# Yujia-Yan/Transkun

Hardware: AMD Instinct MI355X
Metric: semi-CRF logProb+backward steps/sec at T=1024, NBatch=352 (higher is better)
Workload: dtype f32; 1 GPU; NeuralSemiCRFInterval(score, noise).logProb(intervals) fwd+bwd through the public API (Python interval lists packed inside the timed region), T=1024, NBatch=352 per GPU, fp32, exact-hash randn-like scores resident in HBM; T=1024, NBatch=352, impl=0, parallelism=chains sharded, 1 rank(s) seen by the process group, no data-path collective

## Files before the change

transkun_amd/csrc/persist.hip:

```cpp
#include <atomic>
#include <stdlib.h>
#include "common.h"
#include "pathscore.h"

#ifndef SEMICRF_PANEL_PROBES
#define SEMICRF_PANEL_PROBES 0
#endif

#ifndef SEMICRF_PROBE_TASKS
#define SEMICRF_PROBE_TASKS 0
#endif
#ifndef SEMICRF_PROBE_HIST
#define SEMICRF_PROBE_HIST 0
#endif

#ifndef SEMICRF_CT_DBG
#define SEMICRF_CT_DBG -1
#endif

namespace semicrf {

constexpr int PB = 16;
#ifndef SEMICRF_RING
#define SEMICRF_RING 4
// ... 59 lines not shown
constexpr int CTRL_COPYQ = 192;
constexpr int CTRL_PATHQ = 160;
constexpr int CTRL_GEN = 96;

typedef unsigned long long u64;
typedef unsigned v4u __attribute__((ext_vector_type(4)));
typedef unsigned v4u_a4 __attribute__((ext_vector_type(4), aligned(4)));
template <int V>
struct IC { static constexpr int value = V; };

#define DBGF(P) (SEMICRF_CT_DBG >= 0 ? (unsigned)SEMICRF_CT_DBG : (P).dbg)
struct SweepParams {
    const float* score;
    const float* noise;
    int T, B, K;
    int c0, c1;
    int nSpine, nPanelGroups;
    int nTasks;
    int taskBase;
    int panelWaves;
    int hybridPanelWaves;
    int hybridStart;
    int zeroWaves;
    unsigned tag;
    int selfclean;
    unsigned expect_gen;
    unsigned dbg;
    unsigned* ctrl;
    u64* ts;
    unsigned* ug;
    unsigned* ug_other;
    int gradLazyShort;
    int bandWaves;
    u64* farg;
    float* u_out;
    float* last_out;
    int* code;
    const float* vfwd;
    const float* logZ;
    const float* gout;
    int gstride;
    float gscale;
    float* dScore;
    float* dNoise;
    const int* pathPairs;
    const int* pathOffsets;
    int pathK;
    int pathSpine;
    float* pathOut;
    u64* pathg;
    float noiseAdd;
    float* band;
    unsigned* bandFlags;
    int bandSpines;
    int bandGroups;
    int bandK0;
    int copyWaves;
    int cellNT;
    int gradNT;
    int nfarw;
};

__device__ __forceinline__ float fexp2(float x) { return __builtin_amdgcn_exp2f(x); }
__device__ __forceinline__ float flog2(float x) { return __builtin_amdgcn_logf(x); }

__device__ __forceinline__ u64 make_granule(unsigned tag, float v)
// ... 68 lines not shown
}

__device__ __forceinline__ bool spin_abort(unsigned* ctrl, int& spins, int limit, unsigned code)
{
    ++spins;
    if (spins > limit) { set_error(ctrl, code); s_abort = 1; return true; }
    if ((spins & 255) == 0 &&
        __hip_atomic_load(ctrl + 1, __ATOMIC_RELAXED, __HIP_MEMORY_SCOPE_AGENT) != CTRL_INIT) { s_abort = 1; return true; }
    return false;
}

#ifndef SEMICRF_NLOADER
#define SEMICRF_NLOADER 1
#endif
constexpr int NLOADER = SEMICRF_NLOADER;
#ifndef SEMICRF_NRBUF
#define SEMICRF_NRBUF 4
#endif
constexpr int NRBUF = SEMICRF_NRBUF;
constexpr int TILE_BYTES = PB * PB * RS * 4;
constexpr int NCONST = 3;
constexpr int LDS_TILES = 0;
constexpr int LDS_CONST = LDS_TILES + NRBUF * RING * TILE_BYTES;
constexpr int LDS_FAR = LDS_CONST + NRBUF * NCONST * 256;
constexpr int NFAR = 8;
constexpr int NPOS = 128;
static_assert(NFAR >= RING && NPOS >= RING * PB, "ring geometry");
constexpr int LDS_RING = LDS_FAR + NFAR * 64 * 16;
#ifndef SEMICRF_STAGGER
#define SEMICRF_STAGGER 32
#endif
#ifndef SEMICRF_GRAD_LAZY
#define SEMICRF_GRAD_LAZY 127
#endif
#ifndef SEMICRF_GRAD_HSTART
#define SEMICRF_GRAD_HSTART 12
#endif
#ifndef SEMICRF_LOADER_PACE
#define SEMICRF_LOADER_PACE 0
#endif
#ifndef SEMICRF_LOADER_AUX
#define SEMICRF_LOADER_AUX 0
#endif
#ifndef SEMICRF_SPH
#define SEMICRF_SPH 1
#endif
#ifndef SEMICRF_FAR_EARLY
#define SEMICRF_FAR_EARLY 0
#endif
#ifndef SEMICRF_FAR_PRIO
#define SEMICRF_FAR_PRIO 0
#endif
#ifndef SEMICRF_NFARW
#define SEMICRF_NFARW 2
#endif
constexpr int NFARW = SEMICRF_NFARW;
constexpr int NNSLOT = 8;
constexpr int NEAR_SLOT_BYTES = NNEAR * TILE_BYTES + 256;
constexpr int LDS_NEAR = LDS_RING + NPOS * RS * 8;
constexpr int LDS_CTL = LDS_NEAR + (NNEAR > 0 ? NNSLOT * NEAR_SLOT_BYTES : 0);
static_assert(NPOS >= (FAR0 + 1) * PB && NNSLOT >= FAR0 + 1 && NRBUF + RING + NNSLOT + NFARW <= 64 && NNSLOT % NFARW == 0, "near geometry");
constexpr int LDS_DUMMY = LDS_CTL + 256;
constexpr int LDS_SPINE_BYTES = LDS_DUMMY + (64 * 2 + PB * 8) * 4;

typedef __attribute__((address_space(3))) void lds_void_t;
typedef __attribute__((address_space(1))) const void gbl_void_t;
// ... 259 lines not shown
            if (lane == 0) lds_flag_store(fcons, k + 1);
        }
        if (fprobe && k < 64) P.ts[704 + k] = __builtin_amdgcn_s_memrealtime();
        if (NNEAR > 0) {
            const int own0 = k * PB;
            const unsigned bvoff = DIR == 0 ? (unsigned)(((size_t)(prow_c - own0) * T * Bs + cc) * 4)
                                            : (unsigned)(((size_t)(T - 1 - prow_c) * Bs + cc) * 4);
#pragma unroll
            for (int n = NNEAR - 1; n >= 0; --n) {
                const int b = k - RING - n;
                if (b < 0) continue;
                float uq[PB];
#pragma unroll
                for (int u4 = 0; u4 < PB; u4 += 4) {
                    const int j = b * PB + u4;
                    const float* e = rd_base + (j % NPOS) * 8;
                    u64 w0, w1, w2, w3;
                    int spins = 0;
                    while (true) {
                        w0 = lds_load64(e); w1 = lds_load64(e + 2 * RS); w2 = lds_load64(e + 4 * RS); w3 = lds_load64(e + 6 * RS);
                        if (__all((int)(w0 >> 32) == j + 1 && (int)(w1 >> 32) == j + 2 && (int)(w2 >> 32) == j + 3 && (int)(w3 >> 32) == j + 4)) break;
                        __builtin_amdgcn_s_sleep(1);
                        if (spin_abort(ctrl, spins, SPIN_LIMIT_LDS, 12)) break;
                    }
                    uq[u4] = __uint_as_float((unsigned)w0); uq[u4 + 1] = __uint_as_float((unsigned)w1);
                    uq[u4 + 2] = __uint_as_float((unsigned)w2); uq[u4 + 3] = __uint_as_float((unsigned)w3);
                }
                if (fprobe && k < 64 && n == 0) P.ts[768 + k] = __builtin_amdgcn_s_memrealtime();
                if (MODE == 0) {
                    float t[PB];
#pragma unroll
                    for (int u = 0; u < PB; ++u) {
                        t[u] = fmaf(ncell[n][u], LOG2E, uq[u]);
                        if (GRAD && rvalid && P.bandWaves == 0) {
                            const int j = b * PB + u;
                            const size_t co = DIR == 0 ? ((size_t)own0 * T + (size_t)j) * Bs : (size_t)(T - 1 - j) * T * Bs;
                            const auto rs = __builtin_amdgcn_make_buffer_rsrc((void*)(dScore + co), 0, 0x7fffffff, 0x00020000);
                            __builtin_amdgcn_raw_buffer_store_b32(__float_as_uint(gz * fexp2(t[u] + arow)), rs, bvoff, 0, 0);
                        }
                    }
                    float mx = aM;
#pragma unroll
                    for (int u = 0; u < PB; u += 2) mx = fmaxf(mx, fmaxf(t[u], t[u + 1]));
                    float sum = aS * fexp2(aM - mx);
#pragma unroll
                    for (int u = 0; u < PB; ++u) sum += fexp2(t[u] - mx);
                    aM = mx; aS = sum;
                } else {
#pragma unroll
                    for (int u = 0; u < PB; ++u) max_push_sel(aM, aK, uq[u] + ncell[n][u], frame_of<DIR>(b * PB + u, T));
                }
            }
        }
        if (fprobe && k < 64) P.ts[832 + k] = __builtin_amdgcn_s_memrealtime();
        if (rvalid && nparts > 0) {
            for (int p0 = 0; p0 < nparts; p0 += 4) {
                const int np = nparts - p0 < 4 ? nparts - p0 : 4;
                u64 gq[4];
                bool have[4] = {false, false, false, false};
                int spins = 0;
                bool first = SEMICRF_FAR_EARLY && p0 == 0;
                while (true) {
#pragma unroll
                    for (int i = 0; i < 4; ++i)
                        if (i < np && !have[i])
                            gq[i] = first ? eq[i] : load_granule(farg + ((size_t)(p0 + i) * T + prow) * Bs + c);
                    first = false;
// ... 322 lines not shown
            if (GRAD)
                dScore[((size_t)frow * T + frow) * Bs + c] = gz * fexp2(arow + mine + draw - 2.0f * sp);
            if (MODE == 1) code[(size_t)c * T + frow] = (mykey + 1) | (sp > 0.0f ? 0x40000000 : 0);
        }
        if (SEMICRF_PANEL_PROBES && trace) ts[k] = __builtin_amdgcn_s_memrealtime();
    }
}

#ifndef SEMICRF_GRAD_AUX
#define SEMICRF_GRAD_AUX 2
#endif
constexpr int GRAD_AUX = SEMICRF_GRAD_AUX;
#ifndef SEMICRF_CELL_AUX
#define SEMICRF_CELL_AUX 2
#endif
constexpr int CELL_AUX = SEMICRF_CELL_AUX;
#ifndef SEMICRF_PNS
#define SEMICRF_PNS 3
#endif
constexpr int PNS = SEMICRF_PNS;
constexpr int PSTAGE_BYTES = 10240;
#ifndef SEMICRF_PW_MAX
#define SEMICRF_PW_MAX 5
#endif
constexpr int PW_MAX = SEMICRF_PW_MAX;
constexpr int LDS_PANEL_BYTES = PW_MAX * PNS * PSTAGE_BYTES;
constexpr int SPH = SEMICRF_SPH;
constexpr int HWAVES = SPH == 1 ? RING + NLOADER + 1 : RING + NLOADER + NFARW;
constexpr int LDS_HALF = (LDS_SPINE_BYTES + 1023) / 1024 * 1024;
constexpr int LDS_HYBRID_PANEL = SPH * LDS_HALF;
constexpr int HPW_MAX = (160 * 1024 - 512 - LDS_HYBRID_PANEL) / (PNS * PSTAGE_BYTES) < NT / 64 - SPH * HWAVES
                            ? (160 * 1024 - 512 - LDS_HYBRID_PANEL) / (PNS * PSTAGE_BYTES) : NT / 64 - SPH * HWAVES;
static_assert(SPH * HWAVES <= NT / 64 && SPH * LDS_HALF <= 160 * 1024 - 512 && (GP / GS) % SPH == 0, "wave roles");
constexpr int LDS_HYBRID_BYTES = LDS_HYBRID_PANEL + (HPW_MAX > 0 ? HPW_MAX : 0) * PNS * PSTAGE_BYTES;
constexpr int LDS_DYN_MAX2 = SPH * LDS_HALF > LDS_PANEL_BYTES ? SPH * LDS_HALF : LDS_PANEL_BYTES;
constexpr int LDS_DYN_BYTES = LDS_HYBRID_BYTES > LDS_DYN_MAX2 ? LDS_HYBRID_BYTES : LDS_DYN_MAX2;
__device__ __forceinline__ void acc_lift(float& M, float& S, float tm)
{
    const bool need = tm > M + (RESC_HI - RESC_EARLY);
    const float newM = need ? floorf(tm) + RESC_LIFT : M;
    const int sh = (int)fmaxf(M - newM, -4096.0f);
    S = __builtin_ldexpf(S, sh);
    M = newM;
}

struct PanelGeom {
    int pirow[4];
    unsigned voff;
    unsigned fvoff;
    unsigned gvoff;
};

template <int DIR>
__device__ __forceinline__ size_t panel_tile_off(const PanelGeom& G, int m, int T, size_t Bs)
{
    return DIR == 0 ? ((size_t)G.pirow[0] * T + (size_t)m * PB) * Bs
                    : ((size_t)(T - 1 - (m * PB + 15)) * T + (size_t)(T - 1 - G.pirow[3])) * Bs;
}
template <int DIR>
__device__ __forceinline__ unsigned panel_soff(const PanelGeom& G, int rr, int h, int T, size_t Bs)
{
    return DIR == 0 ? (unsigned)((((size_t)(G.pirow[rr] - G.pirow[0]) * T + 8 * h) * Bs) * 4)
                    : (unsigned)((((size_t)(1 - h) * 8 * T + (G.pirow[3] - G.pirow[rr])) * Bs) * 4);
}
template <bool COHERENT>
__device__ __forceinline__ void panel_fetch_gran(__amdgpu_buffer_rsrc_t ursrc, char* stage, unsigned gvoff, int m, int B)
// ... 231 lines not shown
                            else __builtin_amdgcn_s_sleep(SEMICRF_GRAD_LAZY);
                        }
                        else __builtin_amdgcn_s_sleep(16);
                        if (spin_abort(ctrl, spins, SPIN_LIMIT, 5)) break;
                        ++npoll;
                        if (m == q) panel_fetch_gran<true>(ursrc, stage, G.gvoff, m, B);
                        const unsigned pw = __builtin_amdgcn_raw_buffer_load_b32(ursrc, (unsigned)(cl * 4), (unsigned)((m * PB + PB - 1) * B * 4), 16);
                        if (!__all(pw != U_EMPTY || !cvalid)) continue;
                        if (m != q) panel_fetch_gran<true>(ursrc, stage, G.gvoff, m, B);
                        wait_vmcnt<0>();
                        panel_read_gran(grbase + (unsigned)(s * PSTAGE_BYTES), g0, g1);
                    }
                }
                if (frontier && m + 1 < m1) {
                    const int sn = s + 1 == PNS ? 0 : s + 1;
                    panel_fetch_gran<true>(ursrc, stage0 + sn * PSTAGE_BYTES, G.gvoff, m + 1, B);
                    issued += 2;
                    if (sn == 0) mark0 = issued; else if (sn == 1) mark1 = issued; else mark2 = issued;
                }
                if (SEMICRF_PANEL_PROBES && (dbg & 16u) && g == 0 && q4 == 0 && m == q && lane == 0) P.ts[192 + k] = __builtin_amdgcn_s_memrealtime();
                if (c >= c1) { g0.x = 0u; g1.x = 0u; }
                if (c + 1 >= c1) { g0.y = 0u; g1.y = 0u; }
                if (c + 2 >= c1) { g0.z = 0u; g1.z = 0u; }
                if (c + 3 >= c1) { g0.w = 0u; g1.w = 0u; }
                const float uv[2][4] = {{__uint_as_float(g0.x), __uint_as_float(g0.y), __uint_as_float(g0.z), __uint_as_float(g0.w)},
                                        {__uint_as_float(g1.x), __uint_as_float(g1.y), __uint_as_float(g1.z), __uint_as_float(g1.w)}};

                if (MODE == 0) {
                    typedef float v2f __attribute__((ext_vector_type(2)));
                    const v2f l2e = {LOG2E, LOG2E};
                    const v2f u2[2][2] = {{{uv[0][0], uv[0][1]}, {uv[0][2], uv[0][3]}}, {{uv[1][0], uv[1][1]}, {uv[1][2], uv[1][3]}}};
                    const auto gs = __builtin_amdgcn_make_buffer_rsrc((void*)(GRAD ? dScore + panel_tile_off<DIR>(G, m, T, Bs) : nullptr), 0,
                                                                      0x7fffffff, 0x00020000);
#pragma unroll
                    for (int rr = 0; rr < 4; ++rr) {
                        v2f e[2][2];
#pragma unroll
                        for (int h = 0; h < 2; ++h) {
                            const v4u xv = xo[rr * 2 + h];
                            const v2f x2[2] = {{__uint_as_float(xv.x), __uint_as_float(xv.y)}, {__uint_as_float(xv.z), __uint_as_float(xv.w)}};
#pragma unroll
                            for (int j = 0; j < 2; ++j) {
                                const v2f mj = {aM[rr][2 * j], aM[rr][2 * j + 1]};
                                e[h][j] = __builtin_elementwise_fma(x2[j], l2e, u2[h][j] - mj);
                            }
                        }
                        const float emax = fmaxf(fmaxf(fmaxf(e[0][0].x, e[0][0].y), fmaxf(e[0][1].x, e[0][1].y)),
                                                 fmaxf(fmaxf(e[1][0].x, e[1][0].y), fmaxf(e[1][1].x, e[1][1].y)));
                        if (__any(emax > RESC_HI)) {
#pragma unroll
                            for (int i = 0; i < 4; ++i) {
                                const float x0 = __uint_as_float(i == 0 ? xo[rr * 2].x : (i == 1 ? xo[rr * 2].y : (i == 2 ? xo[rr * 2].z : xo[rr * 2].w)));
                                const float x1 = __uint_as_float(i == 0 ? xo[rr * 2 + 1].x : (i == 1 ? xo[rr * 2 + 1].y : (i == 2 ? xo[rr * 2 + 1].z : xo[rr * 2 + 1].w)));
                                const float t0 = fmaf(x0, LOG2E, uv[0][i]), t1 = fmaf(x1, LOG2E, uv[1][i]);
                                acc_lift(aM[rr][i], aS[rr][i], fmaxf(t0, t1));
                                const float e0 = t0 - aM[rr][i], e1 = t1 - aM[rr][i];
                                if (i & 1) { e[0][i >> 1].y = e0; e[1][i >> 1].y = e1; } else { e[0][i >> 1].x = e0; e[1][i >> 1].x = e1; }
                            }
                        }
                        v2f mg[2][2];
#pragma unroll
                        for (int j = 0; j < 2; ++j) {
                            v2f sj = {aS[rr][2 * j], aS[rr][2 * j + 1]};
                            const v2f p0 = {fexp2(e[0][j].x), fexp2(e[0][j].y)};
                            const v2f p1 = {fexp2(e[1][j].x), fexp2(e[1][j].y)};
                            sj = (sj + p0) + p1;
                            aS[rr][2 * j] = sj.x; aS[rr][2 * j + 1] = sj.y;
                            if (GRAD) {
                                const v2f mj = {aM[rr][2 * j], aM[rr][2 * j + 1]};
                                const v2f aj = {arow[rr][2 * j], arow[rr][2 * j + 1]};
                                const v2f fa = mj + aj;
                                const v2f gzj = {gz[2 * j], gz[2 * j + 1]};
                                const v2f fx = {fexp2(fa.x), fexp2(fa.y)};
                                const v2f gF = gzj * fx;
                                mg[0][j] = gF * p0;
                                mg[1][j] = gF * p1;
                            }
                        }
                        if (GRAD) {
#pragma unroll
                            for (int h = 0; h < 2; ++h) {
                                if (cvalid && pbase + rr < T) {
                                    const unsigned so = panel_soff<DIR>(G, rr, h, T, Bs);
                                    v4u gv;
                                    gv.x = __float_as_uint(mg[h][0].x);
                                    gv.y = __float_as_uint(mg[h][0].y);
                                    gv.z = __float_as_uint(mg[h][1].x);
                                    gv.w = __float_as_uint(mg[h][1].y);
#ifdef SEMICRF_NO_PANEL_GSTORE
                                    asm volatile("" ::"v"(gv));
                                    continue;
#endif
                                    if (c + 3 < c1) {
                                        if (grad_nt) __builtin_amdgcn_raw_buffer_store_b128(gv, gs, G.voff, so, GRAD_AUX);
                                        else __builtin_amdgcn_raw_buffer_store_b128(gv, gs, G.voff, so, 0);
                                    }
                                    else {
                                        __builtin_amdgcn_raw_buffer_store_b32(gv.x, gs, G.voff, so, 0);
                                        if (c + 1 < c1) __builtin_amdgcn_raw_buffer_store_b32(gv.y, gs, G.voff + 4, so, 0);
                                        if (c + 2 < c1) __builtin_amdgcn_raw_buffer_store_b32(gv.z, gs, G.voff + 8, so, 0);
                                    }
                                }
                            }
                        }
                        __builtin_amdgcn_sched_barrier(0);
                    }
                    if (GRAD) issued += nst;
                } else {
#pragma unroll
                    for (int rr = 0; rr < 4; ++rr)
#pragma unroll
                        for (int h = 0; h < 2; ++h) {
                            const v4u xv = xo[rr * 2 + h];
                            const float xe[4] = {__uint_as_float(xv.x), __uint_as_float(xv.y), __uint_as_float(xv.z), __uint_as_float(xv.w)};
                            const int key = frame_of<DIR>(m * PB + slot + 8 * h, T);
#pragma unroll
                            for (int i = 0; i < 4; ++i) max_push_seq<DIR>(aM[rr][i], aK[rr][i], uv[h][i] + xe[i], key);
                        }
                }
            }
            if (tprobe) { P.ts[1664 + k] = __builtin_amdgcn_s_memrealtime(); P.ts[1792 + k] = (u64)npoll; }
            if (refill) {
                panel_fetch_cells<DIR>(score, G, stage, m + PNS, T, Bs, cell_nt);
                if (!probe_stream && !probe_nou) panel_fetch_gran<false>(ursrc, stage, G.gvoff, m + PNS, B);
                issued += 10;
                if (s == 0) mark0 = issued; else if (s == 1) mark1 = issued; else mark2 = issued;
            }
        }
        if (tr) { tsp[2] = __builtin_amdgcn_s_memrealtime(); tsp[4] = (u64)(m1 - m0) | ((u64)k << 8) | ((u64)(frontier ? 1 : 0) << 16) | ((u64)part << 20); }
        if (!(GRAD && MODE == 0)) wait_vmcnt<0>();
        (void)frontier;
        if (SEMICRF_PANEL_PROBES && (dbg & 16u) && g == 0 && q4 == 0 && m1 == q + 1 && lane == 0 && k < 64 && T >= 1024)
            P.ts[1728 + k] = __builtin_amdgcn_s_memrealtime();

        const bool b5 = (lane & 32) != 0, b4 = (lane & 16) != 0, b3 = (lane & 8) != 0;
        u64* fbase = farg + (size_t)part * T * Bs;
        const int pi = pbase + (b5 ? 2 : 0) + (b4 ? 1 : 0);
        {
            constexpr int RSTR = 65 * 8;
            char* const rb = stage0;
// ... 54 lines not shown
    if (tail0 + lane < n) rowp[tail0 + lane] = 0.f;
}
__device__ __forceinline__ void zero_role(const SweepParams& P)
{
    const int T = P.T, B = P.B;
    float* const dScore = P.dScore;
    unsigned* const ctrl = P.ctrl;
    const int lane = threadIdx.x & 63;
    const int npairs = T / 2;
    while (true) {
        int p = 0;
        if (lane == 0) p = (int)(atomicAdd(ctrl + 3, 1u) + 1u);
        p = __builtin_amdgcn_readfirstlane(p);
        if (p >= npairs) break;
        const int e2 = T - 2 - p;
        if (p <= e2) zero_row(dScore, p, T, B, lane);
        if (p < e2) zero_row(dScore, e2, T, B, lane);
    }
}

constexpr int CTRL_BANDQ = 32;

template <int DIR>
__device__ __forceinline__ void band_role(const SweepParams& P)
{
    const int T = P.T, B = P.B, K = P.K, c0 = P.c0, c1 = P.c1;
    const size_t Bs = (size_t)B;
    unsigned* const ctrl = P.ctrl;
    const float* __restrict__ score = P.score;
    float* const dScore = P.dScore;
    const int lane = threadIdx.x & 63;
    const int q8 = lane & 7, pjsub = (lane >> 3) & 1, pisub = lane >> 4;
    const int nG = P.nPanelGroups;
    const int nTasks = K * FAR0 * nG * 4;
    const size_t last4 = (size_t)T * T * Bs - 4;
    const auto ursrc = __builtin_amdgcn_make_buffer_rsrc((void*)P.ug, 0, (int)((size_t)T * Bs * 4), 0x00020000);
    const bool grad_nt = __builtin_amdgcn_readfirstlane(P.gradNT) != 0;
    while (true) {
        int task = 0;
        if (lane == 0) task = (int)(atomicAdd(ctrl + CTRL_BANDQ, 1u) + 1u);
        task = __builtin_amdgcn_readfirstlane(task);
        if (task >= nTasks) break;
        const int q4 = task & 3, t2 = task >> 2;
        const int g = t2 % nG, t3 = t2 / nG;
        const int dk = t3 % FAR0, m = t3 / FAR0, k = m + dk;
        const int pbase = k * PB + q4 * 4;
        if (k >= K || pbase >= T) continue;
#if defined(SEMICRF_BAND_ABL) && SEMICRF_BAND_ABL == 2
        continue;
#endif
        const int pi = pbase + pisub;
        const bool rowok = pi < T;
        const int pic = rowok ? pi : T - 1;
        const int c = c0 + g * GP + q8 * 4;
        const int cl = c < c1 ? c : c0;
        const bool v0 = c < c1, v1 = c + 1 < c1, v2 = c + 2 < c1, v3 = c + 3 < c1;
        float gz[4], ar[4];
        {
            const int fr = frame_of<DIR>(pic, T);
#pragma unroll
            for (int i = 0; i < 4; ++i) {
                const bool ok = c + i < c1;
                const float lz = ok ? P.logZ[c + i] : 0.f;
                gz[i] = ok ? P.gout[(size_t)(c + i) * P.gstride] * P.gscale : 0.f;
                ar[i] = ok ? (P.vfwd[(size_t)fr * Bs + c + i] - lz) * LOG2E : 0.f;
            }
        }
        v4u x[8], uu[8];
        size_t off[8];
        unsigned uoff[8];
        bool use[8];
#pragma unroll
        for (int e = 0; e < 8; ++e) {
            const int pj = m * PB + 2 * e + pjsub;
            use[e] = rowok && pj < pi;
            const int pjc = pj < pic ? pj : (pic > 0 ? pic - 1 : 0);
            off[e] = cell_index<DIR>(pic, pjc, T) * Bs + cl;
            uoff[e] = (unsigned)(((size_t)pjc * Bs + cl) * 4);
// ... 91 lines not shown

template <int MODE, int DIR, bool GRAD>
__global__ __launch_bounds__(NT) void persist_sweep_kernel(SweepParams P)
{
    extern __shared__ __attribute__((aligned(16))) char s_dyn[];
    __shared__ int s_exit;
    if (threadIdx.x == 0) {
        const unsigned e1 = __hip_atomic_load(P.ctrl + 1, __ATOMIC_RELAXED, __HIP_MEMORY_SCOPE_AGENT);
        const unsigned gen = P.selfclean ? __hip_atomic_load(P.ctrl + CTRL_GEN, __ATOMIC_RELAXED, __HIP_MEMORY_SCOPE_AGENT) : P.expect_gen;
        s_abort = e1 != CTRL_INIT ? 1 : 0;
        if (gen != P.expect_gen) { set_error(P.ctrl, 13u); s_abort = 1; }
        s_exit = 0;
    }
    for (int h = 0; h < SPH; ++h)
        for (int i = threadIdx.x; i < (LDS_DUMMY - LDS_FAR) / 4; i += NT) ((int*)(s_dyn + h * LDS_HALF + LDS_FAR))[i] = 0;
    __syncthreads();
    const int nSpineWG = (P.nSpine + SPH - 1) / SPH;
    const int ticket = wg_ticket(nSpineWG, (int)gridDim.x, (int)blockIdx.x);
    const int wave = (int)(threadIdx.x >> 6);
    if (P.ug_other && wave == NT / 64 - 1) {
        const size_t n = (size_t)P.T * P.B, n4 = n / 4;
        const size_t per = (n4 + gridDim.x - 1) / gridDim.x, i0 = per * blockIdx.x, i1 = i0 + per < n4 ? i0 + per : n4;
        const v4u e = {U_EMPTY, U_EMPTY, U_EMPTY, U_EMPTY};
        for (size_t i = i0 + (threadIdx.x & 63); i < i1; i += 64) ((v4u*)P.ug_other)[i] = e;
        if (blockIdx.x == 0 && (threadIdx.x & 63) < (int)(n - n4 * 4)) P.ug_other[n4 * 4 + (threadIdx.x & 63)] = U_EMPTY;
    }
    const bool clk = SEMICRF_PANEL_PROBES && (DBGF(P) & 128u) && ticket == nSpineWG + 3 && threadIdx.x == 0;
    if (clk) { P.ts[600] = __builtin_readcyclecounter(); P.ts[601] = __builtin_amdgcn_s_memrealtime(); }
    if (SEMICRF_PROBE_HIST && (DBGF(P) & 1024u) && threadIdx.x == 0) {
        const unsigned long long now = (unsigned long long)__builtin_amdgcn_s_memrealtime();
        atomicMin((unsigned long long*)(P.ts + (3 * P.T) / 2), now);
        atomicMin((unsigned long long*)(P.ts + (3 * P.T) / 2 + 129 + (__builtin_amdgcn_s_getreg(6164) & 7)), now);
    }
    if (ticket < nSpineWG) {
        const int half = wave / HWAVES, hw = wave % HWAVES;
        const int sg = ticket * SPH + half;
        char* const lds_h = s_dyn + half * LDS_HALF;
        if (half >= SPH) {
            const int xw = wave - SPH * HWAVES;
            if (SPH == 1 && NFARW > 1 && wave >= NT / 64 - (NFARW - 1)) {
                if (ticket < P.nSpine && !(DBGF(P) & 9u)) far_role<MODE, DIR, GRAD>(P, ticket, s_dyn, 1 + wave - (NT / 64 - (NFARW - 1)));
            } else if (!(DBGF(P) & 2u) && xw < P.hybridPanelWaves) {
                {
                    const int* cons = (const int*)(s_dyn + LDS_CTL) + NRBUF;
                    int spins = 0;
                    while (lds_flag_load(cons + (P.hybridStart % RING)) < P.hybridStart + 1 && P.hybridStart < P.K &&
                           !(SEMICRF_PANEL_PROBES && (DBGF(P) & 8u))) {
                        __builtin_amdgcn_s_sleep(127);
                        if (spin_abort(P.ctrl, spins, SPIN_LIMIT_LDS, 10)) break;
                    }
                }
                panel_role<MODE, DIR, GRAD>(P, s_dyn + LDS_HYBRID_PANEL, xw, 1);
            } else if (MODE == 0 && DIR == 0 && !GRAD && P.pathPairs != nullptr && P.pathSpine && xw == P.hybridPanelWaves) {
                path_role(P);
            }
        } else if (sg >= P.nSpine) {
        } else if (hw < RING) {
            if (!(DBGF(P) & 8u)) {
                if (GRAD && P.bandWaves == 0) spine_role<MODE, DIR, GRAD, GRAD>(P, sg, hw, lds_h);
                else spine_role<MODE, DIR, GRAD, false>(P, sg, hw, lds_h);
            }
        } else if (hw < RING + NLOADER) {
            if (!(DBGF(P) & 8u)) loader_role<DIR, GRAD>(P, sg, lds_h, hw - RING);
        } else {
            if (!(DBGF(P) & 9u)) far_role<MODE, DIR, GRAD>(P, sg, lds_h, hw - (RING + NLOADER));
        }
    } else {
        if (!(DBGF(P) & 2u) && wave < P.panelWaves)
            panel_role<MODE, DIR, GRAD>(P, s_dyn, wave, 0, P.taskBase > 0 ? (ticket - nSpineWG) * P.panelWaves + wave : -1);
        else if (GRAD && wave - P.panelWaves >= 0 && wave - P.panelWaves < P.zeroWaves) zero_role(P);
        else if (GRAD && wave - P.panelWaves - P.zeroWaves >= 0 && wave - P.panelWaves - P.zeroWaves < P.bandWaves) band_role<DIR>(P);
        else if (SEMICRF_BANDX && wave >= NT / 64 - P.copyWaves && (ticket - nSpineWG) % SEMICRF_BANDX_WGSTRIDE == 0) copy_role<DIR>(P);
        else if (MODE == 0 && DIR == 0 && !GRAD && P.pathPairs != nullptr && wave == P.panelWaves) path_role(P);
    }
    if (clk) { P.ts[602] = __builtin_readcyclecounter(); P.ts[603] = __builtin_amdgcn_s_memrealtime(); }
    if (P.selfclean) {
        int left = 0;
        if ((threadIdx.x & 63) == 0) left = atomicAdd(&s_exit, 1) + 1;
        left = __builtin_amdgcn_readfirstlane(left);
        if (left == NT / 64) {
            unsigned before = 0;
            if ((threadIdx.x & 63) == 0) before = atomicAdd(P.ctrl + CTRL_EXIT, 1u) + 1u;
            before = (unsigned)__builtin_amdgcn_readfirstlane((int)before);
            if (before + 1u == gridDim.x &&
                __hip_atomic_load(P.ctrl + 1, __ATOMIC_RELAXED, __HIP_MEMORY_SCOPE_AGENT) == CTRL_INIT) {
                for (int i = threadIdx.x & 63; i < (int)CTRL_WORDS; i += 64)
                    __hip_atomic_store(P.ctrl + i, i == CTRL_GEN ? P.tag : CTRL_INIT, __ATOMIC_RELAXED, __HIP_MEMORY_SCOPE_AGENT);
            }
        }
    }
}

template <int DIR>
__device__ __forceinline__ void band_copy_load(const float* __restrict__ score, int T, int B, int kr, int g, int t, int q, int lane,
                                               v4u_a4 (&v)[8])
{
    const int q8 = lane & 7, cs = lane >> 3;
    const int cbase = (g * (GP / GS) + q8) * GS;
    const size_t Bs = (size_t)B;
    const size_t last4 = (size_t)T * T * Bs - 4;
    const int kc = kr - t > 0 ? kr - t : 0;
#pragma unroll
    for (int it = 0; it < 8; ++it) {
        const int ci = q * 64 + it * 8 + cs;
        const int col = ci >> 4, tr = ci & 15;
        const int prow_t = kr * PB + tr < T ? kr * PB + tr : T - 1;
        int pj = kc * PB + col;
// ... 134 lines not shown
    static std::atomic<int> ncu[MAX_DEVICES];
    const int dev = current_device();
    int n = ncu[dev].load();
    if (n == 0) {
        int v = 0;
        n = 256;
        if (hipDeviceGetAttribute(&v, hipDeviceAttributeMultiprocessorCount, dev) == hipSuccess && v > 0) n = v;
        ncu[dev].store(n);
    }
    return n;
}

size_t persist_workspace_bytes(int T, int B)
{
    return CTRL_BYTES + align_up((size_t)2 * T * sizeof(u64)) + (size_t)max_parts(T) * align_up((size_t)T * B * sizeof(u64)) +
           2 * align_up((size_t)T * B * sizeof(unsigned)) +
           align_up((size_t)B * sizeof(u64)) +
           band_flag_bytes(T, B) + band_copy_bytes(T, B);
}

bool persist_supported(int T, int B)
{
    return B >= 2 && T >= 2 && T < 65535 && (long long)T * B * 64 < (1ll << 31) &&
           (B + GS - 1) / GS <= MAX_CHUNKS * (device_cus() / 2 > 0 ? device_cus() / 2 : 1);
}

static unsigned next_tag()
{
    static std::atomic<unsigned> counter{0};
    const unsigned lo = (counter.fetch_add(1) % 65534u) + 1u;
    return (lo << 16) | lo;
}

struct Knobs { int hybrid_waves, hybrid_start, panel_waves, zero_waves, band_waves, nfarw; };
static Knobs read_knobs()
{
#if defined(SEMICRF_DEBUG_BUILD) && SEMICRF_DEBUG_BUILD
    auto get = [](const char* name) { const char* e = getenv(name); return e ? atoi(e) : -1; };
    return Knobs{get("SEMICRF_HYBRID_PANEL_WAVES"), get("SEMICRF_HYBRID_START"), get("SEMICRF_PANEL_WAVES"), get("SEMICRF_ZERO_WAVES"),
                 get("SEMICRF_BAND_WAVES"), get("SEMICRF_NFARW_RT")};
#else
    return Knobs{-1, -1, -1, -1, -1, -1};
#endif
}

struct GradArgs {
    const float* vfwd; const float* logZ; const float* gout; float* dScore; float* dNoise; int gstride; float gscale;
    int keep_upper;
    float noise_add;
};
struct PathArgs { const int* pairs; const int* offsets; int K; float* out; };

template <int MODE, int DIR, bool GRAD>
static void launch_one(const SweepParams& P, int grid, hipStream_t stream)
{
    static std::atomic<bool> attr_set[MAX_DEVICES];
    const int dev = current_device();
    if (!attr_set[dev].load()) {
        (void)hipFuncSetAttribute((const void*)persist_sweep_kernel<MODE, DIR, GRAD>,
                                  hipFuncAttributeMaxDynamicSharedMemorySize, LDS_DYN_BYTES);
        attr_set[dev].store(true);
    }
    hipLaunchKernelGGL((persist_sweep_kernel<MODE, DIR, GRAD>), dim3(grid), dim3(NT), LDS_DYN_BYTES, stream, P);
}

static int launch_persist_sweep_impl(int mode, int dir, const float* score, const float* noise, int T, int B,
                                     float* u_out, float* last_out, int* code, void* ws, hipStream_t stream,
                                     const GradArgs* grad, int lease, unsigned lease_tag, const PathArgs* path = nullptr)
{
    SweepParams P;
    P.pathPairs = nullptr; P.pathOffsets = nullptr; P.pathK = 0; P.pathOut = nullptr; P.pathg = nullptr; P.pathSpine = 0; P.noiseAdd = 0.0f;
    P.vfwd = nullptr; P.logZ = nullptr; P.gout = nullptr; P.dScore = nullptr; P.dNoise = nullptr; P.gstride = 1; P.gscale = 1.0f;
    if (grad) {
        P.vfwd = grad->vfwd; P.logZ = grad->logZ; P.gout = grad->gout; P.dScore = grad->dScore; P.dNoise = grad->dNoise;
        P.gstride = grad->gstride; P.gscale = grad->gscale; P.noiseAdd = grad->noise_add;
// ... 57 lines not shown
        int hpw = HPW_MAX > 0 ? HPW_MAX : 0;
        if (knobs.hybrid_waves >= 0 && knobs.hybrid_waves <= HPW_MAX) hpw = knobs.hybrid_waves;
        int hstart = grad ? SEMICRF_GRAD_HSTART : P.K * 5 / 8;
        hstart = hstart < 8 ? 8 : (hstart > 40 ? 40 : hstart);
        if (knobs.hybrid_start >= 0) hstart = knobs.hybrid_start;
        P.hybridStart = hstart;
        P.hybridPanelWaves = hpw;
        int pw = (T >= 1024 && nb >= 256) ? PW_MAX : (PW_MAX < 4 ? PW_MAX : 4);
        if (knobs.panel_waves > 0) pw = knobs.panel_waves;
        if (pw < 1) pw = 1;
        if (pw > PW_MAX) pw = PW_MAX;
        P.panelWaves = pw;
        int zw = 0;
        if (grad && ci == 0 && !grad->keep_upper) {
            zw = 2;
            if (knobs.zero_waves >= 0) zw = knobs.zero_waves;
            if (zw > NT / 64 - pw) zw = NT / 64 - pw;
            if (nPanelWG <= 0 || P.nTasks == 0) zw = 0;
            if (zw == 0 && T > 1) {
                launch_zero_upper(grad->dScore, T, B, stream);
            }
        }
        P.zeroWaves = zw;
        int bw = 0;
        if (grad && nPanelWG > 0 && P.nTasks > 0) {
            bw = 3;
            if (knobs.band_waves >= 0) bw = knobs.band_waves;
            if (bw > NT / 64 - pw - zw) bw = NT / 64 - pw - zw;
        }
        P.bandWaves = bw;
        P.gradLazyShort = nb < 256 ? 1 : 0;
        P.nfarw = (!grad && nb <= SEMICRF_NFARW2_MAXB && T >= SEMICRF_NFARW2_MINT && NFARW >= 2) ? 2 : 1;
        if (knobs.nfarw >= 1 && knobs.nfarw <= NFARW) P.nfarw = knobs.nfarw;
        P.cellNT = cell_policy_nt(T, B, SEMICRF_NT_MIN_MB) ? 1 : 0;
        if (!SEMICRF_NT_MISALIGNED && grad && B % 32 != 0) P.cellNT = 0;
        P.gradNT = cell_policy_nt(T, B, SEMICRF_GRAD_NT_MIN_MB) ? 1 : 0;
        if (P.nTasks == 0) nPanelWG = 0;
        P.pathSpine = nPanelWG == 0 ? 1 : 0;
        P.band = nullptr; P.copyWaves = 0;
        if (band_ok && !grad && nchunks == 1 && nPanelWG > 0 && NT / 64 - pw - zw - bw - 1 >= SEMICRF_BANDX_WAVES) {
            P.bandFlags = (unsigned*)(w + band_off);
            P.band = (float*)(w + band_off + band_flag_bytes(T, B));
            P.bandK0 = SEMICRF_BANDX_K0;
            P.copyWaves = SEMICRF_BANDX_WAVES;
        }
        const int grid = nSpineWG + nPanelWG;
        P.taskBase = nPanelWG * P.panelWaves;
        if (P.taskBase > P.nTasks) P.taskBase = P.nTasks;
        if (grad) launch_one<0, 1, true>(P, grid, stream);
        else if (mode == 0 && dir == 0) launch_one<0, 0, false>(P, grid, stream);
        else if (mode == 0 && dir == 1) launch_one<0, 1, false>(P, grid, stream);
        else if (mode == 1 && dir == 0) launch_one<1, 0, false>(P, grid, stream);
        else launch_one<1, 1, false>(P, grid, stream);
    }
    return 0;
}

int launch_persist_sweep(int mode, int dir, const float* score, const float* noise, int T, int B, float* u_out,
                         float* last_out, int* code, void* ws, hipStream_t stream, int lease, unsigned lease_tag)
{
    return launch_persist_sweep_impl(mode, dir, score, noise, T, B, u_out, last_out, code, ws, stream, nullptr, lease, lease_tag);
}

int launch_persist_logprob_fwd(const float* score, const float* noise, int T, int B, float* u_out, float* logZ, const int* pairs,
                               int K, const int* offsets, float* logProb, void* ws, hipStream_t stream, int lease, unsigned lease_tag)
{
// ... 42 lines not shown
```

Baseline: 1914 steps/s.

## Run band gradient work on spare spine-workgroup waves and allow extending band depth

Adds spine-band waves: spare waves in spine workgroups wait until the hybrid panel start has been consumed, then execute band_role alongside the panel workgroups' band waves, so more waves share the band gradient work. It also adds a bandExtra knob that widens the band task set (more diagonal offsets) and drops panel-side marginal gradient stores for those tiles. bandExtra defaults to 0, so by default only the extra spine band waves (default 2) take effect. This moves band-gradient work onto otherwise idle waves, at the cost of more concurrent memory traffic and contention on the shared task counter.

```diff
diff --git a/transkun_amd/csrc/persist.hip b/transkun_amd/csrc/persist.hip
--- a/transkun_amd/csrc/persist.hip
+++ b/transkun_amd/csrc/persist.hip
@@ -115,6 +115,8 @@
     unsigned* ug_other;
     int gradLazyShort;
     int bandWaves;
+    int spineBandWaves;
+    int bandExtra;
     u64* farg;
     float* u_out;
     float* last_out;
@@ -249,6 +251,12 @@
 #endif
 #ifndef SEMICRF_GRAD_LAZY
 #define SEMICRF_GRAD_LAZY 127
+#endif
+#ifndef SEMICRF_SPINE_BAND_WAVES
+#define SEMICRF_SPINE_BAND_WAVES 2
+#endif
+#ifndef SEMICRF_BAND_EXTRA
+#define SEMICRF_BAND_EXTRA 0
 #endif
 #ifndef SEMICRF_GRAD_HSTART
 #define SEMICRF_GRAD_HSTART 12
@@ -574,7 +582,7 @@
 #pragma unroll
                     for (int u = 0; u < PB; ++u) {
                         t[u] = fmaf(ncell[n][u], LOG2E, uq[u]);
-                        if (GRAD && rvalid && P.bandWaves == 0) {
+                        if (GRAD && rvalid && P.bandWaves + P.spineBandWaves == 0) {
                             const int j = b * PB + u;
                             const size_t co = DIR == 0 ? ((size_t)own0 * T + (size_t)j) * Bs : (size_t)(T - 1 - j) * T * Bs;
                             const auto rs = __builtin_amdgcn_make_buffer_rsrc((void*)(dScore + co), 0, 0x7fffffff, 0x00020000);
@@ -963,6 +971,8 @@
 constexpr int HPW_MAX = (160 * 1024 - 512 - LDS_HYBRID_PANEL) / (PNS * PSTAGE_BYTES) < NT / 64 - SPH * HWAVES
                             ? (160 * 1024 - 512 - LDS_HYBRID_PANEL) / (PNS * PSTAGE_BYTES) : NT / 64 - SPH * HWAVES;
 static_assert(SPH * HWAVES <= NT / 64 && SPH * LDS_HALF <= 160 * 1024 - 512 && (GP / GS) % SPH == 0, "wave roles");
+static_assert(HPW_MAX + 1 + (SPH == 1 ? NFARW - 1 : 0) <= NT / 64 - SPH * HWAVES,
+              "the streaming, path, far and band waves of a spine workgroup do not fit its spare waves");
 constexpr int LDS_HYBRID_BYTES = LDS_HYBRID_PANEL + (HPW_MAX > 0 ? HPW_MAX : 0) * PNS * PSTAGE_BYTES;
 constexpr int LDS_DYN_MAX2 = SPH * LDS_HALF > LDS_PANEL_BYTES ? SPH * LDS_HALF : LDS_PANEL_BYTES;
 constexpr int LDS_DYN_BYTES = LDS_HYBRID_BYTES > LDS_DYN_MAX2 ? LDS_HYBRID_BYTES : LDS_DYN_MAX2;
@@ -1260,6 +1270,11 @@
                     const v2f u2[2][2] = {{{uv[0][0], uv[0][1]}, {uv[0][2], uv[0][3]}}, {{uv[1][0], uv[1][1]}, {uv[1][2], uv[1][3]}}};
                     const auto gs = __builtin_amdgcn_make_buffer_rsrc((void*)(GRAD ? dScore + panel_tile_off<DIR>(G, m, T, Bs) : nullptr), 0,
                                                                       0x7fffffff, 0x00020000);
+#ifdef SEMICRF_FRONTIER_NOMARG
+                    const bool marg = GRAD && m < q;
+#else
+                    const bool marg = GRAD && m <= q - __builtin_amdgcn_readfirstlane(P.bandExtra);
+#endif
 #pragma unroll
                     for (int rr = 0; rr < 4; ++rr) {
                         v2f e[2][2];
@@ -1294,7 +1309,7 @@
                             const v2f p1 = {fexp2(e[1][j].x), fexp2(e[1][j].y)};
                             sj = (sj + p0) + p1;
                             aS[rr][2 * j] = sj.x; aS[rr][2 * j + 1] = sj.y;
-                            if (GRAD) {
+                            if (GRAD && marg) {
                                 const v2f mj = {aM[rr][2 * j], aM[rr][2 * j + 1]};
                                 const v2f aj = {arow[rr][2 * j], arow[rr][2 * j + 1]};
                                 const v2f fa = mj + aj;
@@ -1305,7 +1320,7 @@
                                 mg[1][j] = gF * p1;
                             }
                         }
-                        if (GRAD) {
+                        if (GRAD && marg) {
 #pragma unroll
                             for (int h = 0; h < 2; ++h) {
                                 if (cvalid && pbase + rr < T) {
@@ -1333,7 +1348,7 @@
                         }
                         __builtin_amdgcn_sched_barrier(0);
                     }
-                    if (GRAD) issued += nst;
+                    if (GRAD && marg) issued += nst;
                 } else {
 #pragma unroll
                     for (int rr = 0; rr < 4; ++rr)
@@ -1454,7 +1469,8 @@
     const int lane = threadIdx.x & 63;
     const int q8 = lane & 7, pjsub = (lane >> 3) & 1, pisub = lane >> 4;
     const int nG = P.nPanelGroups;
-    const int nTasks = K * FAR0 * nG * 4;
+    const int ndk = FAR0 + __builtin_amdgcn_readfirstlane(P.bandExtra);
+    const int nTasks = K * ndk * nG * 4;
     const size_t last4 = (size_t)T * T * Bs - 4;
     const auto ursrc = __builtin_amdgcn_make_buffer_rsrc((void*)P.ug, 0, (int)((size_t)T * Bs * 4), 0x00020000);
     const bool grad_nt = __builtin_amdgcn_readfirstlane(P.gradNT) != 0;
@@ -1465,7 +1481,7 @@
         if (task >= nTasks) break;
         const int q4 = task & 3, t2 = task >> 2;
         const int g = t2 % nG, t3 = t2 / nG;
-        const int dk = t3 % FAR0, m = t3 / FAR0, k = m + dk;
+        const int dk = t3 % ndk, m = t3 / ndk, k = m + dk;
         const int pbase = k * PB + q4 * 4;
         if (k >= K || pbase >= T) continue;
 #if defined(SEMICRF_BAND_ABL) && SEMICRF_BAND_ABL == 2
@@ -1623,13 +1639,24 @@
         atomicMin((unsigned long long*)(P.ts + (3 * P.T) / 2), now);
         atomicMin((unsigned long long*)(P.ts + (3 * P.T) / 2 + 129 + (__builtin_amdgcn_s_getreg(6164) & 7)), now);
     }
+    bool do_band = false;
     if (ticket < nSpineWG) {
         const int half = wave / HWAVES, hw = wave % HWAVES;
         const int sg = ticket * SPH + half;
         char* const lds_h = s_dyn + half * LDS_HALF;
         if (half >= SPH) {
             const int xw = wave - SPH * HWAVES;
-            if (SPH == 1 && NFARW > 1 && wave >= NT / 64 - (NFARW - 1)) {
+            const int sb1 = NT / 64 - (P.nfarw - 1), sb0 = sb1 - P.spineBandWaves;
+            if (GRAD && SPH == 1 && wave >= sb0 && wave < sb1) {
+                const int* cons = (const int*)(s_dyn + LDS_CTL) + NRBUF;
+                int spins = 0;
+                bool gone = false;
+                while (lds_flag_load(cons + (P.hybridStart % RING)) < P.hybridStart + 1 && P.hybridStart < P.K) {
+                    __builtin_amdgcn_s_sleep(127);
+                    if (spin_abort(P.ctrl, spins, SPIN_LIMIT_LDS, 17)) { gone = true; break; }
+                }
+                do_band = !gone;
+            } else if (SPH == 1 && NFARW > 1 && wave >= NT / 64 - (NFARW - 1)) {
                 if (ticket < P.nSpine && !(DBGF(P) & 9u)) far_role<MODE, DIR, GRAD>(P, ticket, s_dyn, 1 + wave - (NT / 64 - (NFARW - 1)));
             } else if (!(DBGF(P) & 2u) && xw < P.hybridPanelWaves) {
                 {
@@ -1648,7 +1675,7 @@
         } else if (sg >= P.nSpine) {
         } else if (hw < RING) {
             if (!(DBGF(P) & 8u)) {
-                if (GRAD && P.bandWaves == 0) spine_role<MODE, DIR, GRAD, GRAD>(P, sg, hw, lds_h);
+                if (GRAD && P.bandWaves + P.spineBandWaves == 0) spine_role<MODE, DIR, GRAD, GRAD>(P, sg, hw, lds_h);
                 else spine_role<MODE, DIR, GRAD, false>(P, sg, hw, lds_h);
             }
         } else if (hw < RING + NLOADER) {
@@ -1660,10 +1687,11 @@
         if (!(DBGF(P) & 2u) && wave < P.panelWaves)
             panel_role<MODE, DIR, GRAD>(P, s_dyn, wave, 0, P.taskBase > 0 ? (ticket - nSpineWG) * P.panelWaves + wave : -1);
         else if (GRAD && wave - P.panelWaves >= 0 && wave - P.panelWaves < P.zeroWaves) zero_role(P);
-        else if (GRAD && wave - P.panelWaves - P.zeroWaves >= 0 && wave - P.panelWaves - P.zeroWaves < P.bandWaves) band_role<DIR>(P);
+        else if (GRAD && wave - P.panelWaves - P.zeroWaves >= 0 && wave - P.panelWaves - P.zeroWaves < P.bandWaves) do_band = true;
         else if (SEMICRF_BANDX && wave >= NT / 64 - P.copyWaves && (ticket - nSpineWG) % SEMICRF_BANDX_WGSTRIDE == 0) copy_role<DIR>(P);
         else if (MODE == 0 && DIR == 0 && !GRAD && P.pathPairs != nullptr && wave == P.panelWaves) path_role(P);
     }
+    if (GRAD && do_band) band_role<DIR>(P);
     if (clk) { P.ts[602] = __builtin_readcyclecounter(); P.ts[603] = __builtin_amdgcn_s_memrealtime(); }
     if (P.selfclean) {
         int left = 0;
@@ -1864,15 +1892,15 @@
     return (lo << 16) | lo;
 }
 
-struct Knobs { int hybrid_waves, hybrid_start, panel_waves, zero_waves, band_waves, nfarw; };
+struct Knobs { int hybrid_waves, hybrid_start, panel_waves, zero_waves, band_waves, nfarw, spine_band_waves, band_extra; };
 static Knobs read_knobs()
 {
 #if defined(SEMICRF_DEBUG_BUILD) && SEMICRF_DEBUG_BUILD
     auto get = [](const char* name) { const char* e = getenv(name); return e ? atoi(e) : -1; };
     return Knobs{get("SEMICRF_HYBRID_PANEL_WAVES"), get("SEMICRF_HYBRID_START"), get("SEMICRF_PANEL_WAVES"), get("SEMICRF_ZERO_WAVES"),
-                 get("SEMICRF_BAND_WAVES"), get("SEMICRF_NFARW_RT")};
+                 get("SEMICRF_BAND_WAVES"), get("SEMICRF_NFARW_RT"), get("SEMICRF_SPINE_BAND_WAVES"), get("SEMICRF_BAND_EXTRA_RT")};
 #else
-    return Knobs{-1, -1, -1, -1, -1, -1};
+    return Knobs{-1, -1, -1, -1, -1, -1, -1, -1};
 #endif
 }
 
@@ -1996,6 +2024,19 @@
         P.gradLazyShort = nb < 256 ? 1 : 0;
         P.nfarw = (!grad && nb <= SEMICRF_NFARW2_MAXB && T >= SEMICRF_NFARW2_MINT && NFARW >= 2) ? 2 : 1;
         if (knobs.nfarw >= 1 && knobs.nfarw <= NFARW) P.nfarw = knobs.nfarw;
+        int sbw = 0, bx = 0;
+        if (grad && SPH == 1 && nPanelWG > 0 && P.nTasks > 0) {
+            sbw = SEMICRF_SPINE_BAND_WAVES;
+            if (knobs.spine_band_waves >= 0) sbw = knobs.spine_band_waves;
+            const int room = NT / 64 - SPH * HWAVES - hpw - (P.nfarw - 1);
+            if (sbw > room) sbw = room;
+            if (sbw < 0) sbw = 0;
+            bx = SEMICRF_BAND_EXTRA;
+            if (knobs.band_extra >= 0 && knobs.band_extra <= 2) bx = knobs.band_extra;
+            if (bw + sbw == 0) bx = 0;
+        }
+        P.spineBandWaves = sbw;
+        P.bandExtra = bx;
         P.cellNT = cell_policy_nt(T, B, SEMICRF_NT_MIN_MB) ? 1 : 0;
         if (!SEMICRF_NT_MISALIGNED && grad && B % 32 != 0) P.cellNT = 0;
         P.gradNT = cell_policy_nt(T, B, SEMICRF_GRAD_NT_MIN_MB) ? 1 : 0;
```

New measurement: 1870 steps/s. 0.977x the previous value.
